# CogSP/CoEvoNet

Measured on AMD Instinct MI355X. Metric: env-steps/sec (agent-steps of the whole job; generations/sec in gens_per_sec), Co-GA simple_adversary_v3 pop=200 HoF=5, higher is better.
Workload: dtype f32

## Files before the change

coevonet_amd/csrc/fc_forward.hip:

```cpp
#include <cstdlib>
#include <type_traits>

#include "coevo_common.hip.h"

namespace coevo {

#ifndef COEVO_HEAVY16_U
#define COEVO_HEAVY16_U 4
#endif
#ifndef COEVO_LIGHT_U
#define COEVO_LIGHT_U 8
#endif

typedef float f32x4_t __attribute__((ext_vector_type(4)));
typedef float f32x4_acc __attribute__((ext_vector_type(4)));
__device__ inline float4 load_stream16(const float4 *p)
{
#ifdef COEVO_NO_NT
    return *p;
#else
    const f32x4_t v = __builtin_nontemporal_load(reinterpret_cast<const f32x4_t *>(p));
    return make_float4(v[0], v[1], v[2], v[3]);
#endif
}
// ... 1054 lines not shown
template <int NB>
__device__ __forceinline__ float mfma16_row_total(const float (*red)[8], int lc, int lg)
{
    const float *rr = red[4 * lg + (lc & 3)];
    const float4 a = *reinterpret_cast<const float4 *>(rr);
    float tot = ((a.x + a.y) + a.z) + a.w;
    if constexpr (NB == 8) {
        const float4 b = *reinterpret_cast<const float4 *>(rr + 4);
        tot = (((tot + b.x) + b.y) + b.z) + b.w;
    }
    return tot;
}
__device__ __forceinline__ void quad_spread(float v, float (&out)[4])
{
    out[0] = dpp_move<0x00>(v); out[1] = dpp_move<0x55>(v); out[2] = dpp_move<0xAA>(v); out[3] = dpp_move<0xFF>(v);
}

template <int MODE>
__device__ __forceinline__ void fc_policy_mfma16_body(const FcArgs &a, FcMfma16Smem &sm, const coevo_fc_task &task)
{
    typedef unsigned u32x2_s __attribute__((ext_vector_type(2)));
    COEVO_STAMP(0);
    const int t = threadIdx.x, w = t >> 6, l = t & 63, lc = l & 15, lg = l >> 4;
    const int D = task.D, nrows = task.n_rows, row0 = task.row_begin;
    const float *net = a.slab + task.net_off;
    int st = 0;

    constexpr int KS = 3;
    float *par = &sm.h1a[0][0];
    {
        const int n_pieces = (D + 3) * (H1 / 4);
#pragma unroll
        for (int j = 0; j < 7; ++j)
            if (64 * w + 256 * j < n_pieces)
                __builtin_amdgcn_global_load_lds((const __attribute__((address_space(1))) void *)(net + 4 * (t + 256 * j)),
                                                 (__attribute__((address_space(3))) void *)(par + 4 * (64 * w + 256 * j)),
                                                 16, 0, 0);
    }
    float p_b2[4], p_g2[4], p_be2[4];
    {
        const float *b2p = net + fc_off_b2(D);
#pragma unroll
        for (int T = 0; T < 4; ++T) p_b2[T] = b2p[64 * w + 16 * T + lc];
    }
    const float p_b3 = (t < 16 * NACT) ? net[fc_off_b3(D) + t % NACT] : 0.0f;

    if constexpr (MODE >= MODE_FUSED) {
// ... 81 lines not shown
        for (int T = 0; T < 8; ++T) c1[T][i] = c1[T][i] - stat[i];
    }
    mfma16_block_sums<8, true>(c1, l, s1);
    mfma16_post_sums<8>(s1, sm.red, w, lc, lg);
    __syncthreads();
    quad_spread(1.0f / __builtin_sqrtf(mfma16_row_total<8>(sm.red, lc, lg) * (1.0f / H1) + LN_EPS), stat);
#pragma unroll
    for (int i = 0; i < 4; ++i) {
        const int row = 4 * lg + i;
        const float rstd = stat[i];
#pragma unroll
        for (int T = 0; T < 8; ++T) {
            const float y = __builtin_fmaf(c1[T][i] * rstd, p_g1[T], p_be1[T]);
            if (row < nrows && bad_post_relu(y)) st |= COEVO_ST_BAD_FC1;
            const int k = 128 * w + 16 * T + lc;
            sm.h1a[k][row ^ ((k >> 2) & 3)] = relu_keep_nan(y);
        }
    }
    asm volatile("" : "+v"(st));
    __syncthreads();
    COEVO_STAMP(2);

    f32x4_acc c2[4];
    {
#pragma unroll
        for (int T = 0; T < 4; ++T)
#pragma unroll
            for (int i = 0; i < 4; ++i) c2[T][i] = p_b2[T];
        const float4 *wp = reinterpret_cast<const float4 *>(net + fc_off_w2(D)) + (size_t)w * 128 * 64 + l;
        constexpr int U = COEVO_HEAVY16_U;
        float4 bufA[U], bufB[U];
        auto issue = [&](float4 (&buf)[U], int kq) {
#pragma unroll
            for (int u = 0; u < U; ++u) buf[u] = wp[(size_t)(kq + u) * 64];
        };
        auto consume = [&](const float4 (&buf)[U], int kq) {
#pragma unroll
            for (int u = 0; u < U; ++u) {
                const int q = kq + u;
                const float av = sm.h1a[4 * q + lg][lc ^ (q & 3)];
                const u32x2_s s02 = __builtin_amdgcn_permlane32_swap(__float_as_uint(buf[u].x), __float_as_uint(buf[u].z), false, false);
                const u32x2_s s13 = __builtin_amdgcn_permlane32_swap(__float_as_uint(buf[u].y), __float_as_uint(buf[u].w), false, false);
                const u32x2_s y01 = __builtin_amdgcn_permlane16_swap(s02[0], s13[0], false, false);
                const u32x2_s y23 = __builtin_amdgcn_permlane16_swap(s02[1], s13[1], false, false);
                c2[0] = __builtin_amdgcn_mfma_f32_16x16x4f32(av, __uint_as_float(y01[0]), c2[0], 0, 0, 0);
                c2[1] = __builtin_amdgcn_mfma_f32_16x16x4f32(av, __uint_as_float(y01[1]), c2[1], 0, 0, 0);
                c2[2] = __builtin_amdgcn_mfma_f32_16x16x4f32(av, __uint_as_float(y23[0]), c2[2], 0, 0, 0);
                c2[3] = __builtin_amdgcn_mfma_f32_16x16x4f32(av, __uint_as_float(y23[1]), c2[3], 0, 0, 0);
            }
        };
        issue(bufA, 0);
        int kq = 0;
        for (; kq < 128 - 2 * U; kq += 2 * U) {
            issue(bufB, kq + U);
            __builtin_amdgcn_sched_barrier(0);
            consume(bufA, kq);
            issue(bufA, kq + 2 * U);
            __builtin_amdgcn_sched_barrier(0);
            consume(bufB, kq + U);
        }
        issue(bufB, kq + U);
        __builtin_amdgcn_sched_barrier(0);
        consume(bufA, kq);
        consume(bufB, kq + U);
    }
    COEVO_STAMP(3);
    float s2[1];
    mfma16_block_sums<4, false>(c2, l, s2);
    mfma16_post_sums<4>(s2, sm.red, w, lc, lg);
    __syncthreads();
    quad_spread(mfma16_row_total<4>(sm.red, lc, lg) * (1.0f / H2), stat);
    __syncthreads();
#pragma unroll
    for (int i = 0; i < 4; ++i) {
#pragma unroll
        for (int T = 0; T < 4; ++T) c2[T][i] = c2[T][i] - stat[i];
    }
    mfma16_block_sums<4, true>(c2, l, s2);
    mfma16_post_sums<4>(s2, sm.red, w, lc, lg);
    __syncthreads();
    quad_spread(1.0f / __builtin_sqrtf(mfma16_row_total<4>(sm.red, lc, lg) * (1.0f / H2) + LN_EPS), stat);
#pragma unroll
    for (int i = 0; i < 4; ++i) {
        const int row = 4 * lg + i;
        const float rstd = stat[i];
#pragma unroll
        for (int T = 0; T < 4; ++T) {
            const float y = __builtin_fmaf(c2[T][i] * rstd, p_g2[T], p_be2[T]);
// ... 668 lines not shown
```

coevonet_amd/csrc/offspring.hip:

```cpp
#include "coevo_common.hip.h"
#include "dqn_common.hip.h"
#include "promote_roles.hip.h"
#include "philox.hip.h"

namespace coevo {

__device__ inline void slab_quad_normals(uint64_t seed, uint32_t slo, uint32_t shi, int64_t s0, int D, int64_t P,
                                         float z[4])
{
    int64_t p[4];
#pragma unroll
    for (int i = 0; i < 4; ++i) p[i] = (s0 + i < P) ? fc_slab_to_flat(s0 + i, D) : -1;
    float zz[4];
    int64_t have = -1;
#pragma unroll
    for (int i = 0; i < 4; ++i) {
        if (p[i] < 0) { z[i] = 0.0f; continue; }
        const int64_t q = p[i] >> 2;
        if (q != have) { philox_normal4(seed, slo, shi, (uint32_t)q, zz); have = q; }
        z[i] = zz[p[i] & 3];
    }
}

__device__ __forceinline__ void fc_perturb_block(const float *parent_slab, const int32_t *parent_idx, float *child_slab,
// ... 191 lines not shown
__global__ __launch_bounds__(256) void ga_promote_kernel(GaPromoteArgs a)
{
    const unsigned y = blockIdx.y;
    const PromoteRole R = PROMOTE_ROLE(a, y);
    float *pop = static_cast<float *>(R.pop), *hof = static_cast<float *>(R.hof), *elite = static_cast<float *>(R.elite);
    const int64_t stride = fc_stride(R.D);
    const int64_t s0 = ((int64_t)blockIdx.x * 256 + threadIdx.x) * 4;
    if (s0 >= stride) return;
    float4 e0;
    if (a.sigma && !R.from_pop) {
        uint32_t shi = a.stream_hi_prev + y;
        if (a.gen_dev) shi += 4u * (uint32_t)(*a.gen_dev - 1);
        e0 = promote_rebuild<0>(elite, R.order, stride, s0, a.E, R.D, a.sigma[y], a.seed, shi);
    } else {
        e0 = R.from_pop ? promote_elites<0>(pop, R.order, elite, stride, s0, a.E)
                        : *reinterpret_cast<const float4 *>(elite + s0);
    }
    promote_hof_shift<1>(hof, stride, s0, a.hof);
    *reinterpret_cast<float4 *>(hof + (int64_t)(a.hof - 1) * stride + s0) = e0;
    if (R.to_pop0) *reinterpret_cast<float4 *>(pop + s0) = e0;
    if (a.tick && blockIdx.x == 0 && blockIdx.y == 0 && threadIdx.x == 0) *a.tick += 1;
}

__device__ __forceinline__ float4 es_chunk_sum(float4 tv, const float *pp, int64_t stride, const float *fitness, int lo, int hi)
{
    const float th[4] = {tv.x, tv.y, tv.z, tv.w};
    float acc[4] = {0.0f, 0.0f, 0.0f, 0.0f};
    typedef float f32x4_nt __attribute__((ext_vector_type(4)));
    constexpr int UE = 16;
    int i = lo;
    for (; i + UE <= hi; i += UE) {
        float4 pv[UE];
#pragma unroll
        for (int u = 0; u < UE; ++u) {
            const f32x4_nt v = __builtin_nontemporal_load(reinterpret_cast<const f32x4_nt *>(pp + (int64_t)(i + u) * stride));
            pv[u] = make_float4(v[0], v[1], v[2], v[3]);
        }
#pragma unroll
        for (int u = 0; u < UE; ++u) {
            const float f = fitness[i + u];
            acc[0] = __builtin_fmaf(f, pv[u].x - th[0], acc[0]);
            acc[1] = __builtin_fmaf(f, pv[u].y - th[1], acc[1]);
            acc[2] = __builtin_fmaf(f, pv[u].z - th[2], acc[2]);
            acc[3] = __builtin_fmaf(f, pv[u].w - th[3], acc[3]);
        }
    }
// ... 224 lines not shown
{
    GaPromoteArgs a{};
    if (!promote_roles(a, roles, n_roles, E, hof, false)) return COEVO_ERR_ARG;
    a.sigma = sigma; a.seed = seed; a.stream_hi_prev = stream_hi_prev; a.gen_dev = gen_dev; a.tick = tick;
    unsigned max_blocks = 0;
    for (int r = 0; r < n_roles; ++r) max_blocks = std::max(max_blocks, quad_blocks(fc_stride(roles[r].D)));
    hipLaunchKernelGGL(ga_promote_kernel, dim3(max_blocks, (unsigned)n_roles), dim3(256), 0, (hipStream_t)stream, a);
    COEVO_HIP_CHECK(hipGetLastError());
    return COEVO_OK;
}

extern "C" int coevo_ga_promote(const coevo_ga_promote_role *roles, int n_roles, int E, int hof, void *stream)
{
    return ga_promote_launch(roles, n_roles, E, hof, nullptr, 0, 0, nullptr, nullptr, stream);
}

extern "C" int coevo_ga_promote_tick(const coevo_ga_promote_role *roles, int n_roles, int E, int hof, int32_t *counter,
                                     void *stream)
{
    if (!counter) return COEVO_ERR_ARG;
    return ga_promote_launch(roles, n_roles, E, hof, nullptr, 0, 0, nullptr, counter, stream);
}

extern "C" int coevo_ga_promote_rebuild(const coevo_ga_promote_role *roles, int n_roles, int E, int hof, const float *sigma,
                                        uint64_t seed, uint32_t stream_hi_prev, const int32_t *gen_dev, void *stream)
{
    if (!sigma) return COEVO_ERR_ARG;
    for (int r = 0; roles && r < n_roles && r < 3; ++r)
        if (!roles[r].elites_from_pop && !roles[r].order) return COEVO_ERR_ARG;
    return ga_promote_launch(roles, n_roles, E, hof, sigma, seed, stream_hi_prev, gen_dev, nullptr, stream);
}

extern "C" int coevo_es_update(float *theta_slab_net, const float *pert_slab, int D, const float *fitness, int n,
                               const float *sigma_dev, float lr, void *stream)
{
    if (!theta_slab_net || !pert_slab || !fitness || !sigma_dev || !fc_dim_ok(D) || n <= 0) return COEVO_ERR_ARG;
    const dim3 grid(quad_blocks(fc_stride(D)));
    hipLaunchKernelGGL(es_update_kernel, grid, dim3(256), 0, (hipStream_t)stream, theta_slab_net, pert_slab, D,
                       fitness, n, sigma_dev, lr);
    COEVO_HIP_CHECK(hipGetLastError());
    return COEVO_OK;
}

static int es_partial_launch(const float *theta_net, const float *pert_slab_local, int ind_first, int64_t stride,
                             const float *fitness_all, int n_total, int chunks_total, int chunk_first, int n_chunks,
                             float *partial, void *stream)
// ... 115 lines not shown
```

coevonet_amd/genetic_algorithm.py:

```python
from __future__ import annotations

import os
import time

import numpy as np
import torch

from . import lib as L
from .fcnetwork import FCNetwork
from .ga_half import HalfGAEngine
from .game_logic import create_agent
from .mpe.simple_adversary import ENV_SEED
from .population import (N_EVAL, RET_SLOT, ROLE_D, ROLES, SIGMA_ATTR, CoGASchedule, CoGATail, NetTable, SlabIO,
                         adapt_mutation_power, captured, co_ga_games, eval_gate_limits, half_route, mean_eval_triple,
                         shard_and_gather, slab_layout)
from .rollout import DeviceRollout, HostEnvRollout, RolloutPlan, effective_steps

ROLE_SLOT = {"agent_0": 1, "agent_1": 2, "adversary_0": 0}


def evaluate_current_weights(agent_0, agent_1, adversary, env, args):
    from .game_logic import play_game
    tot = [0.0, 0.0, 0.0]
    for _ in range(N_EVAL):
# ... 9 lines not shown
    children = []
    for i in range(args.population - 1):
        child = elites[i % args.elites_number].clone(env, args, role)
        child.mutate(sigma)
        children.append(child)
    return children


def small_shard_rows(n_local, hof, cus, pop):
    if n_local >= pop or not 1 <= hof <= 8:
        return 16
    per_cu = 2 if os.environ.get("COEVO_PERSISTENT", "1") != "0" else 1
    if 3 * n_local + 6 * hof * -(-n_local // hof) <= per_cu * cus:
        return hof
    return 16


def cohort_partition(n_local, K):
    bounds = np.array([k * n_local // K for k in range(K + 1)], dtype=np.int64)
    return bounds, np.searchsorted(bounds[1:], np.arange(n_local), side="right").astype(np.int32)


RESIDENT_MB_DEFAULT = 224


def resident_budget_bytes():
    v = os.environ.get("COEVO_RESIDENT_MB", "").strip().lower()
    if v == "all":
        return float("inf")
    return (float(v) if v else RESIDENT_MB_DEFAULT) * 1e6


def resident_enabled(env, heavy_rows, n_local, pop):
    return env == "device" and heavy_rows == 16 and n_local >= pop


def resident_prefix(budget_bytes, fixed_bytes, individual_bytes, bounds):
    K = len(bounds) - 1
    sizes = np.diff(np.asarray(bounds, dtype=np.int64))
    left = budget_bytes - fixed_bytes
    if left <= 0 or K <= 0:
        return np.zeros(K, dtype=np.int64)
    if left == float("inf"):
        return sizes
    return np.minimum(sizes, int(left // (K * individual_bytes)))

# ... 9 lines not shown
                 env_seed=ENV_SEED, rng="device_philox", philox_seed=0, env="device", first_ordinal=1,
                 shard=(0, 1), gather=None, timing_pairs=4096, cohorts=1, gather_packed=None):
        assert 1 <= elites <= pop and hof >= 1
        self.pop, self.hof, self.E = pop, hof, elites
        self.rng_mode, self.philox_seed, self.env_mode = rng, int(philox_seed), env
        self.device = device
        self.rank, self.world = shard
        self.gather = gather
        self.gather_packed = gather_packed
        if self.world > 1 and pop % self.world:
            raise ValueError(f"population {pop} is not divisible by the number of ranks {self.world}")
        self.lo = self.rank * pop // self.world
        self.hi = (self.rank + 1) * pop // self.world
        self.n_local = self.hi - self.lo
        self.T_train = effective_steps(limit_train, max_cycles)
        self.T_eval = effective_steps(limit_eval, max_cycles)
        self.n_cycles = (max(self.T_train, self.T_eval) + 2) // 3
        self.first_ordinal = first_ordinal
        self.env_seed = env_seed
        self.stride = {r: L.fc_slab_stride(ROLE_D[r]) for r in ROLES}
        self.P = {r: L.fc_param_count(ROLE_D[r]) for r in ROLES}
        self.base, total = slab_layout(ROLES, (("pop", pop), ("hof", hof), ("elite", elites), ("stale", 1), ("hof_tmp", hof),
                                               ("elite_prev", elites)), self.stride)
        self.slab = torch.zeros(total, dtype=torch.float32, device=device)
        table = NetTable(self.base, self.stride, ROLE_D)
        games, self.n_main = co_ga_games(table, self.lo, self.hi, hof)
        heavy_rows = int(os.environ.get("COEVO_HEAVY_ROWS", "0"))
        if heavy_rows <= 0:
            cus = torch.cuda.get_device_properties(device).multi_processor_count if (env == "device" and str(device) != "cpu") else 0
            heavy_rows = small_shard_rows(self.n_local, hof, cus, pop) if (cus and cohorts <= 1) else 16
        host_k = int(os.environ.get("COEVO_HOST_COHORTS", "0")) or max(1, min(4, len(games) // 700))
        self.K = max(1, min(int(cohorts) if env == "device" else host_k, self.n_local))
        row_order = "class" if env == "device" else "cohort"
        self._set_cohort_bounds()
        game_cohort = None
        if self.K > 1:
            per_ind = np.repeat(cohort_partition(self.n_local, self.K)[1], self.hof)
            game_cohort = np.concatenate([per_ind, per_ind, per_ind, np.full(N_EVAL, self.K - 1)]).astype(np.int32)
        resident = resident_enabled(env, heavy_rows, self.n_local, pop)

        def resident_nets():
            if not resident:
                return ()
            ind_bytes = sum(4 * self.stride[r] for r in ROLES)
            n = resident_prefix(resident_budget_bytes(), (hof + elites + 1) * ind_bytes, ind_bytes, self.cohort_bounds)
            return [table.ids[("pop", r, self.lo + i)] for r in ROLES for k in range(self.K)
                    for i in range(int(self.cohort_bounds[k]), int(self.cohort_bounds[k]) + int(n[k]))]

        try:
            self.plan = RolloutPlan(np.array(games), table.net_off, table.net_D, device=device, heavy_rows=heavy_rows,
                                    n_cohorts=self.K, game_cohort=game_cohort, row_order=row_order,
                                    resident_nets=resident_nets())
        except ValueError:
            self.K = 1
            self._set_cohort_bounds()
            self.plan = RolloutPlan(np.array(games), table.net_off, table.net_D, device=device, heavy_rows=heavy_rows,
                                    row_order=row_order, resident_nets=resident_nets())
        if env == "device":
            self.ro = DeviceRollout(self.plan, self.slab, env_seed=env_seed, timing_pairs=timing_pairs)
        else:
            self.ro = HostEnvRollout(self.plan, self.slab, env_seed=env_seed)
        f32 = dict(dtype=torch.float32, device=device)
        self.dist_all = torch.zeros(3, pop, **f32)
        self.dist = {r: self.dist_all[i] for i, r in enumerate(ROLES)}
        self.div = {r: torch.zeros(1, **f32) for r in ROLES}
        self.fitness = {r: torch.zeros(pop, **f32) for r in ROLES}
        self.order = {r: torch.zeros(pop, dtype=torch.int32, device=device) for r in ROLES}
        self.sigma = {r: torch.zeros(1, **f32) for r in ROLES}
        self.sigma_prev = {r: torch.zeros(1, **f32) for r in ROLES}
        self.last_reward = torch.zeros(3, pop, 3, dtype=torch.float64, device=device)
        self.pack_local = torch.zeros(3, self.n_local, 4, dtype=torch.float64, device=device)
        self.pack_all = torch.zeros(self.world, 3, self.n_local, 4, dtype=torch.float64, device=device)
        self.parent_idx = torch.tensor([c % elites for c in range(max(pop - 1, 1))], dtype=torch.int32, device=device)
        self.hof_shift_idx = torch.arange(1, max(hof, 2), dtype=torch.int32, device=device)
        self.iota = torch.arange(max(hof, elites, 2), dtype=torch.int32, device=device)
        self.generation = 0
        self.steps_per_generation = 3 * pop * hof * self.T_train + N_EVAL * self.T_eval

    def _uploaded(self, region):
        if region in ("pop", "stale"):
            self._dist_current = False

    def download(self, role, region, first, n):
        if region == "pop":
            self.flush_breeding()
        return super().download(role, region, first, n)

    def eval_rewards(self):
        self.ro.check_status()
        if hasattr(self.ro, "collect_stamps"):
            self.ro.collect_stamps()
        return mean_eval_triple(self.rewards_host()[self.n_main:])

    def select(self):
        if torch.is_tensor(self.ro.rewards):
            dev_rewards = self.ro.rewards
        else:
            if getattr(self, "_rewards_dev", None) is None:
                self._rewards_pin = torch.zeros(self.plan.n_games, 3, dtype=torch.float64).pin_memory()
                self._rewards_dev = torch.zeros(self.plan.n_games, 3, dtype=torch.float64, device=self.device)
            self._rewards_pin.numpy()[:] = self.ro.rewards
            self._rewards_dev.copy_(self._rewards_pin, non_blocking=True)
            dev_rewards = self._rewards_dev
        per_phase = self.n_local * self.hof
# ... 177 lines not shown
        if tick:
            L.call("coevo_counter_add", L._p(self.gen_dev), 1)

    def _reset_cohort(self, k, gen):
        lo_k, hi_k = self._cohort_individuals(k)
        base, M = self._ordinal_base(gen), 3 * self.pop * self.hof
        per_phase = self.n_local * self.hof
        segs = [(ph * per_phase + (lo_k - self.lo) * self.hof, (hi_k - lo_k) * self.hof,
                 base + ph * self.pop * self.hof + lo_k * self.hof) for ph in range(3)]
        if k == self.K - 1 and gen > 0:
            segs.append((self.n_main, N_EVAL, self._ordinal_base(gen - 1) + M))
        self.ro.reset_segments(segs, arm=(k, self.n_cycles))

    def flush_breeding(self):
        if getattr(self, "_breeding_pending", False):
            torch.cuda.synchronize()
            for k in range(self.K):
                self._breed_cohort(k, self.generation_enqueued - 1)
            torch.cuda.synchronize()
            self._breeding_pending = False

    def replay_generation_pipelined(self, gen):
        assert self.world == 1 and self.env_mode == "device" and self.fused_tail and self.K > 1
        self._enqueue_cohort_chains(gen)
        if self._tail_graph is None:
            self._tail_graph = captured(lambda: self._enqueue_selection_and_breeding(breed=False))
        self._tail_graph.replay()
        self._breeding_pending = self.pop > 1
        self.generation_enqueued = gen + 1

    def _enqueue_cohort_chains(self, gen):
        ro = self.ro
        if gen <= 1:
            ro.set_limits(eval_gate_limits(self.plan.n_games, self.n_main, self.T_train, self.T_eval, gen))
        main = torch.cuda.current_stream()
        if getattr(self, "_cohort_streams", None) is None:
            self._cohort_streams = [main] + [
                torch.cuda.ExternalStream(L.load().coevo_rollout_ctx_cohort_stream(ro.ctx, k), device=self.device)
                for k in range(1, self.K)]
            self._cohort_done = [torch.cuda.Event() for _ in range(self.K)]
            self._tail_done = torch.cuda.Event()
            self._tail_graph = None
            self._breeding_pending = False
        self._tail_done.record(main)
        for k, s in reversed(list(enumerate(self._cohort_streams))):
            if k:
# ... 353 lines not shown
```

coevonet_amd/lib.py:

```python
from __future__ import annotations

import ctypes as C
import os

import numpy as np
import torch

HERE = os.path.dirname(os.path.abspath(__file__))
LIB_PATH = os.environ.get("COEVO_LIB") or os.path.join(HERE, "libcoevo.so")

OBS_STRIDE = 12
LOGIT_STRIDE = 8
FC_MAX_ROWS = 32
MPE_STATE_DOUBLES = 24
STAMP_SLOTS = 32
ST_NAMES = {1: "input contains inf or NaN", 2: "output contains inf or NaN after fc1",
            4: "output contains inf or NaN after fc2", 8: "output contains inf or NaN",
            16: "no action selected (current_best_position = -1)",
            32: "persistent rollout: a workgroup timed out waiting for the other rows of its games (COEVO_ST_SYNC_TIMEOUT)",
            64: "fp16 forward: a task with a bad width, row count or unaligned net offset was skipped (COEVO_ST_BAD_TASK)"}

DQN_LOGIT_STRIDE = 32
DQN_FC1_TILED = 0x100
DQP_SKIP_BN = 1
DQN_MAX_ROWS = 16
DQN_TASK_DTYPE = np.dtype([("net_off", "<i8"), ("row_begin", "<i4"), ("n_rows", "<i4")])

TASK_DTYPE = np.dtype([("net_off", "<i8"), ("row_begin", "<i4"), ("n_rows", "<i4"), ("D", "<i4"),
                       ("reserved", "<i4")])
TASK_RESIDENT = 1


class PCG64State(C.Structure):
    _fields_ = [("state_hi", C.c_uint64), ("state_lo", C.c_uint64), ("inc_hi", C.c_uint64), ("inc_lo", C.c_uint64)]

    @classmethod
    def from_seed(cls, seed):
        st = np.random.PCG64(seed).state["state"]
        m = (1 << 64) - 1
        return cls(st["state"] >> 64, st["state"] & m, st["inc"] >> 64, st["inc"] & m)


class PerturbJob(C.Structure):
    _fields_ = [("parent_slab", C.c_void_p), ("parent_idx", C.c_void_p), ("child_slab", C.c_void_p),
                ("sigma_dev", C.c_void_p), ("dist_ref", C.c_void_p), ("dist_partial", C.c_void_p),
                ("child_first", C.c_int32), ("n_children", C.c_int32), ("D", C.c_int32),
                ("stream_lo_first", C.c_uint32), ("stream_hi", C.c_uint32), ("pad", C.c_int32)]


class Perturb16Job(C.Structure):
    _fields_ = list(PerturbJob._fields_)


# ... 101 lines not shown
    "coevo_fc16_distance": (C.c_int, [C.c_void_p, C.c_void_p, C.c_int, C.c_int, C.c_void_p, C.c_void_p]),
    "coevo_fc16_distance_finalize": (C.c_int, [C.c_void_p, C.c_int, C.c_int, C.c_void_p, C.c_int, C.c_void_p,
                                               C.c_void_p]),
    "coevo_fc16_perturb_dist_multi": (C.c_int, [C.c_void_p, C.c_int, C.c_uint64, C.c_int, C.c_void_p, C.c_void_p]),
    "coevo_fc16_distance_finalize_multi": (C.c_int, [C.c_void_p, C.c_int, C.c_void_p]),
    "coevo_fc16_gather": (C.c_int, [C.c_void_p, C.c_void_p, C.c_void_p, C.c_int, C.c_int, C.c_int, C.c_void_p]),
    "coevo_ga16_promote": (C.c_int, [C.c_void_p, C.c_int, C.c_int, C.c_int, C.c_void_p]),
    "coevo_es16_partial_floats": (C.c_int64, [C.c_int]),
    "coevo_es16_fitness": (C.c_int, [C.c_void_p, C.c_void_p, C.c_int, C.c_int, C.c_void_p, C.c_void_p, C.c_void_p]),
    "coevo_es16_partial": (C.c_int, [C.c_int, C.c_void_p, C.c_int, C.c_int, C.c_void_p, C.c_uint64, C.c_uint32, C.c_uint32,
                                     C.c_void_p, C.c_void_p]),
    "coevo_es16_apply": (C.c_int, [C.c_void_p, C.c_void_p, C.c_int, C.c_int, C.c_int, C.c_void_p, C.c_double, C.c_void_p]),
    "coevo_fc_forward_merged": (C.c_int, [C.c_void_p, C.c_void_p, C.c_int, C.c_int, C.c_void_p, C.c_int, C.c_int, C.c_void_p,
                                         C.c_void_p, C.c_void_p, C.c_void_p, C.c_void_p]),
    "coevo_mpe_reset": (C.c_int, [C.c_void_p, C.c_int, C.c_int, C.c_int, PCG64State, C.c_uint64, C.c_void_p]),
    "coevo_mpe_reset_multi": (C.c_int, [C.c_void_p, C.c_int, C.c_void_p, C.c_int, PCG64State, C.c_void_p]),
    "coevo_mpe_reset_multi_arm": (C.c_int, [C.c_void_p, C.c_int, C.c_void_p, C.c_int, PCG64State, C.c_void_p, C.c_int,
                                            C.c_void_p]),
    "coevo_mpe_reset_multi_prep": (C.c_int, [C.c_void_p, C.c_int, C.c_void_p, C.c_int, PCG64State, C.c_void_p, C.c_int,
                                             C.c_void_p, C.c_int, C.c_void_p]),
    "coevo_ga_select_adapt": (C.c_int, [C.c_void_p, C.c_int, C.c_int, C.c_int, C.c_int, C.c_void_p, C.c_int, C.c_void_p,
                                        C.c_void_p]),
    "coevo_ga_promote_tick": (C.c_int, [C.c_void_p, C.c_int, C.c_int, C.c_int, C.c_void_p, C.c_void_p]),
    "coevo_fc_perturb_dist_multi": (C.c_int, [C.c_void_p, C.c_int, C.c_uint64, C.c_int, C.c_void_p, C.c_void_p]),
    "coevo_fc_distance_finalize_multi": (C.c_int, [C.c_void_p, C.c_int, C.c_void_p]),
    "coevo_mpe_reset_gen": (C.c_int, [C.c_void_p, C.c_int, C.c_int, C.c_int, PCG64State, C.c_int64, C.c_void_p,
                                      C.c_int64, C.c_void_p]),
    "coevo_mpe_observe": (C.c_int, [C.c_void_p, C.c_int, C.c_void_p, C.c_void_p, C.c_int, C.c_void_p, C.c_void_p]),
    "coevo_mpe_step": (C.c_int, [C.c_void_p, C.c_int, C.c_void_p, C.c_void_p, C.c_int, C.c_void_p, C.c_int,
                                 C.c_void_p]),
    "coevo_mpe_host_reset": (C.c_int, [C.c_void_p, C.c_int, PCG64State, C.c_void_p]),
    "coevo_mpe_host_reset_games": (C.c_int, [C.c_void_p, C.c_int, PCG64State, C.c_void_p, C.c_void_p, C.c_int, C.c_int]),
    "coevo_mpe_host_observe": (C.c_int, [C.c_void_p, C.c_int, C.c_void_p, C.c_void_p, C.c_int, C.c_void_p]),
    "coevo_mpe_host_step": (C.c_int, [C.c_void_p, C.c_int, C.c_void_p, C.c_void_p, C.c_int, C.c_int, C.c_void_p, C.c_int]),
    "coevo_mpe_host_step_games": (C.c_int, [C.c_void_p, C.c_int, C.c_void_p, C.c_void_p, C.c_int, C.c_void_p, C.c_int,
                                            C.c_void_p, C.c_int, C.c_int, C.c_int, C.c_void_p]),
    "coevo_host_rollout_create": (C.c_void_p, [C.c_int, C.c_int]),
    "coevo_host_rollout_destroy": (None, [C.c_void_p]),
    "coevo_host_rollout_threads": (C.c_int, [C.c_void_p]),
    "coevo_host_rollout_step": (C.c_int, [C.c_void_p, C.c_void_p, C.c_int, C.c_void_p, C.c_void_p, C.c_int, C.c_int,
                                          C.c_void_p, C.c_int, C.c_void_p, C.c_int, C.c_int, C.c_void_p]),
    "coevo_mpe_host_rollout": (C.c_int, [C.c_void_p, C.POINTER(HostRolloutDesc), C.c_void_p]),
    "coevo_host_placement_choose": (C.c_int, [C.c_char_p, C.c_char_p, C.c_char_p, C.c_char_p, C.c_int, C.c_int, C.c_int,
                                              C.c_void_p, C.c_void_p]),
    "coevo_host_rollout_placement": (C.c_int, [C.c_void_p, C.c_void_p, C.c_int, C.c_void_p]),
    "coevo_host_rollout_alloc": (C.c_void_p, [C.c_void_p, C.c_size_t]),
# ... 222 lines not shown
```

coevonet_amd/population.py:

```python
from __future__ import annotations

import os

import numpy as np
import torch

from . import lib as L
from .rollout import DeviceRollout, RolloutPlan

ROLES = ("agent_0", "agent_1", "adversary_0")
ROLE_D = {"agent_0": 10, "agent_1": 10, "adversary_0": 8}
RET_SLOT = {"agent_0": 0, "agent_1": 1, "adversary_0": 2}
ROLES2 = ("first_0", "second_0")
N_EVAL = 10
ES_CHUNKS = 8
SIGMA_ATTR = {"agent_0": "mutation_power_agent_0", "agent_1": "mutation_power_agent_1",
              "adversary_0": "mutation_power_adversary"}


def slab_layout(roles, regions, stride_of):
    base, off = {}, 0
    for r in roles:
        base[r] = {}
        for region, count in regions:
# ... 198 lines not shown
    _perturb_dist_entry = "coevo_fc_perturb_dist"
    _finalize_entry = "coevo_fc_distance_finalize"

    def _select_roles(self, rewards_ptr_of, game_first_of, games_per_individual):
        roles = (L.GaSelectRole * 3)()
        for ri, r in enumerate(ROLES):
            roles[ri] = L.GaSelectRole(L._p(self.dist[r]), rewards_ptr_of(ri), L._p(self.div[r]), L._p(self.fitness[r]),
                                       L._p(self.order[r]), L._p(self.best_dist[r]), game_first_of(ri), RET_SLOT[r])
        L.call("coevo_ga_select", roles, 3, self.pop, games_per_individual, self.hof)

    def _select_unfused(self, rewards_ptr_of, game_first_of, games_per_individual):
        for ri, r in enumerate(ROLES):
            L.call("coevo_sharing_score", L._p(self.dist[r]), self.pop, L._p(self.div[r]))
            L.call("coevo_ga_fitness", rewards_ptr_of(ri), game_first_of(ri), self.pop, games_per_individual, self.hof,
                   RET_SLOT[r], L._p(self.div[r]), L._p(self.fitness[r]))
            L.call("coevo_rank_desc", L._p(self.fitness[r]), self.pop, L._p(self.order[r]))

    def _promote_roles(self, elites_from_pop, best_to_pop0, tick=False, rebuild=None):
        roles = (L.GaPromoteRole * 3)()
        for ri, r in enumerate(ROLES):
            roles[ri] = L.GaPromoteRole(self._ptr(r, "pop"), self._ptr(r, "hof"), self._ptr(r, "elite"),
                                        L._p(self.order[r]), ROLE_D[r], 1 if elites_from_pop else 0,
                                        1 if best_to_pop0 else 0, 0)
        if rebuild is not None:
            L.call("coevo_ga_promote_rebuild", roles, 3, self.E, self.hof, L._p(self.sigma32_prev), self.philox_seed, *rebuild)
        elif tick:
            L.call("coevo_ga_promote_tick", roles, 3, self.E, self.hof, L._p(self.gen_dev))
        else:
            L.call(self._promote_entry, roles, 3, self.E, self.hof)

    def _elites_unfused(self, r, rebuild=None):
        D = ROLE_D[r]
        if rebuild is None:
            L.call("coevo_fc_gather", self._ptr(r, "pop"), L._p(self.order[r]), self._ptr(r, "elite"), 0, self.E, D)
            return
        sigma_ptr, stream, gen_ptr = rebuild
        L.call("coevo_fc_gather", self._ptr(r, "elite"), L._p(self.iota), self._ptr(r, "elite_prev"), 0, self.E, D)
        L.call("coevo_fc_rebuild_elites", self._ptr(r, "elite_prev"), L._p(self.order[r]), self._ptr(r, "elite"), self.E, D,
               sigma_ptr, self.philox_seed, stream, gen_ptr)

    def _hof_push(self, r):
        D = ROLE_D[r]
        if self.hof > 1:
            L.call("coevo_fc_gather", self._ptr(r, "hof"), L._p(self.hof_shift_idx), self._ptr(r, "hof_tmp"), 0,
                   self.hof - 1, D)
            L.call("coevo_fc_gather", self._ptr(r, "hof_tmp"), L._p(self.iota), self._ptr(r, "hof"), 0,
                   self.hof - 1, D)
        L.call("coevo_fc_gather", self._ptr(r, "elite"), L._p(self.iota), self._ptr(r, "hof"), self.hof - 1, 1, D)

    def _best_to_pop0(self, r):
        L.call("coevo_fc_gather", self._ptr(r, "elite"), L._p(self.iota), self._ptr(r, "pop"), 0, 1, ROLE_D[r])

    def _promote_unfused(self, r, best_to_pop0=True, best_dist=False):
        self._hof_push(r)
        if best_to_pop0:
            self._best_to_pop0(r)
        if best_dist:
            L.call("coevo_gather_f32", L._p(self.best_dist[r]), L._p(self.dist[r]), L._p(self.order[r]), 1)

    def _breed_role_children(self, ri, r, c_lo, c_hi, stream, gen_dev, sigma_ptr):
        L.call(self._perturb_dist_entry, self._ptr(r, "elite"), self.parent_idx.data_ptr() + 4 * c_lo, self._ptr(r, "pop"),
               1 + c_lo, c_hi - c_lo, ROLE_D[r], sigma_ptr, self.philox_seed, c_lo, stream, 0, gen_dev, self._ptr(r, "stale"),
               L._p(self.dist_partial[r]))
        L.call(self._finalize_entry, L._p(self.dist_partial[r]), self.pblocks[r], c_hi - c_lo, L._p(self.dist[r]), 1 + c_lo,
               L._p(self.best_dist[r]) if c_lo == 0 else None)


class CoESSchedule:

    def _rollout_pair(self, games, eval_games, table, env_seed, cls=DeviceRollout, host_cohorts=None, **ro_kw):
        cohorts = int(os.environ.get("COEVO_ES_COHORTS", "2")) if host_cohorts is None else host_cohorts
# ... 145 lines not shown
```

include/coevo.h:

```cpp
#ifndef COEVO_H
#define COEVO_H

#include <stddef.h>
#include <stdint.h>

#ifdef __cplusplus
extern "C" {
#endif

#define COEVO_VERSION 103

#define COEVO_OK 0
#define COEVO_ERR_ARG (-1)
#define COEVO_ERR_HIP (-2)
#define COEVO_ERR_UNSUPPORTED (-3)

#define COEVO_ST_BAD_INPUT 1
#define COEVO_ST_BAD_FC1 2
#define COEVO_ST_BAD_FC2 4
#define COEVO_ST_BAD_OUT 8
#define COEVO_ST_NO_ACTION 16
#define COEVO_ST_SYNC_TIMEOUT 32
#define COEVO_ST_BAD_TASK 64

// ... 5 lines not shown
#define COEVO_FC_MAX_ROWS 32
#define COEVO_STAMP_SLOTS 32

#define COEVO_SLOT_ADVERSARY 0
#define COEVO_SLOT_AGENT_0 1
#define COEVO_SLOT_AGENT_1 2

int coevo_version(void);
const char *coevo_build_flags(void);

int64_t coevo_fc_param_count(int D);
int64_t coevo_fc_slab_stride(int D);
int coevo_fc_pack(const float *flat, float *slab, int n, int D, void *stream);
int coevo_fc_unpack(const float *slab, float *flat, int n, int D, void *stream);

typedef struct {
    int64_t net_off;
    int32_t row_begin;
    int32_t n_rows;
    int32_t D;
    int32_t reserved;
} coevo_fc_task;
#define COEVO_TASK_RESIDENT 1

int coevo_fc_forward_argmax(const float *slab, const coevo_fc_task *tasks, int n_tasks, int max_rows_per_task,
                            const float *obs, int32_t *actions, float *logits, int32_t *status, void *stream);
int coevo_fc_forward_merged(const float *slab, const coevo_fc_task *heavy_tasks, int n_heavy, int heavy_max_rows,
                            const coevo_fc_task *light_tasks, int n_light, int light_max_rows, const float *obs,
                            int32_t *actions, float *logits, int32_t *status, void *stream);

int64_t coevo_fc16_slab_stride(int D);
int coevo_fc16_pack(const float *flat, void *slab, int n, int D, void *stream);
int coevo_fc16_unpack(const void *slab, float *flat, int n, int D, void *stream);
int coevo_fc16_forward_argmax(const void *slab, const coevo_fc_task *tasks, int n_tasks, int max_rows_per_task,
                              const float *obs, int32_t *actions, float *logits, int32_t *status, void *stream);

#define COEVO_MPE_STATE_DOUBLES 24
typedef struct {
    uint64_t pcg_state_hi, pcg_state_lo, pcg_inc_hi, pcg_inc_lo;
} coevo_pcg64;

int coevo_mpe_reset(double *state, int n_games, int game_first, int count, coevo_pcg64 rng, uint64_t first_ordinal,
                    void *stream);
typedef struct { int32_t game_first, count; uint64_t first_ordinal; } coevo_reset_seg;
int coevo_mpe_reset_multi(double *state, int n_games, const coevo_reset_seg *segs , int n_segs,
                          coevo_pcg64 rng, void *stream);
// ... 193 lines not shown
    float *fitness;
    int32_t *order;
    float *best_dist;
    int32_t game_first;
    int32_t slot;
} coevo_ga_select_role;
int coevo_ga_select(const coevo_ga_select_role *roles, int n_roles, int pop, int games_per_individual, int hof,
                    void *stream);
int coevo_ga_select_gathered(const coevo_ga_select_role *roles, int n_roles, int pop, int hof, const double *gathered,
                             int n_local, void *stream);
typedef struct coevo_ga_adapt_args {
    const double *rewards; const int32_t *gen_dev; double *hist; double *sig_hist; double *sigma64; float *sigma32;
    float *sigma32_prev; double sig_min, sig_max; int32_t eval_first_game, cap, adaptive, reserved;
} coevo_ga_adapt_args;
int coevo_ga_select_adapt(const coevo_ga_select_role *roles, int n_roles, int pop, int games_per_individual, int hof,
                          const double *gathered, int n_local, const coevo_ga_adapt_args *adapt, void *stream);
typedef struct coevo_ga_promote_role {
    float *pop, *hof, *elite;
    const int32_t *order;
    int32_t D, elites_from_pop, best_to_pop0, reserved;
} coevo_ga_promote_role;
int coevo_ga_promote(const coevo_ga_promote_role *roles, int n_roles, int E, int hof, void *stream);
int coevo_ga_promote_tick(const coevo_ga_promote_role *roles, int n_roles, int E, int hof, int32_t *counter, void *stream);
int coevo_ga_promote_rebuild(const coevo_ga_promote_role *roles, int n_roles, int E, int hof, const float *sigma,
                             uint64_t seed, uint32_t stream_hi_prev, const int32_t *gen_dev, void *stream);
int coevo_fc_gather(const float *src_slab, const int32_t *src_idx, float *dst_slab, int dst_first, int n, int D,
                    void *stream);

int64_t coevo_fc16_perturb_blocks(int D);
int coevo_fc16_perturb_dist(const void *parent_slab, const int32_t *parent_idx, void *child_slab, int child_first,
                            int n_children, int D, const float *sigma_dev, uint64_t seed, uint32_t stream_lo_first,
                            uint32_t stream_hi, int flags, const int32_t *gen_dev, const void *dist_ref,
                            double *dist_partial, void *stream);
int coevo_fc16_distance(const void *ref_net, const void *pop_slab, int n, int D, double *dist_partial, void *stream);
int coevo_fc16_distance_finalize(const double *dist_partial, int n_blocks, int n, float *dist, int first, const float *head,
                                 void *stream);
typedef struct {
    const void *parent_slab; const int32_t *parent_idx; void *child_slab; const float *sigma_dev;
    const void *dist_ref; double *dist_partial;
    int32_t child_first, n_children, D; uint32_t stream_lo_first, stream_hi; int32_t pad;
} coevo_fc16_perturb_job;
int coevo_fc16_perturb_dist_multi(const coevo_fc16_perturb_job *jobs , int n_jobs, uint64_t seed, int flags,
                                  const int32_t *gen_dev, void *stream);
int coevo_fc16_distance_finalize_multi(const coevo_fc_finalize_job *jobs , int n_jobs, void *stream);
int coevo_fc16_gather(const void *src_slab, const int32_t *src_idx, void *dst_slab, int dst_first, int n, int D, void *stream);
typedef struct coevo_ga16_promote_role {
// ... 145 lines not shown
```

Before: 150.0 million.

## Keep tile-major twin copies of hall-of-fame FC2 weights to skip lane permutes

Adds a second copy of each hall-of-fame net's FC2 weight matrix, stored in a tile-major order that matches the MFMA operand layout. Heavy forward tasks that evaluate HoF nets are flagged to read this twin, so they feed MFMAs directly and skip the permlane32/permlane16 swap sequence. The twins are kept in sync by a new promote kernel that shifts them alongside the HoF, plus refresh calls on other update paths. This costs extra device memory, extra writes during promotion and more bookkeeping, and any update path that misses a refresh would read stale weights.

```diff
diff --git a/coevonet_amd/csrc/fc_forward.hip b/coevonet_amd/csrc/fc_forward.hip
--- a/coevonet_amd/csrc/fc_forward.hip
+++ b/coevonet_amd/csrc/fc_forward.hip
@@ -1100,7 +1100,7 @@
     typedef unsigned u32x2_s __attribute__((ext_vector_type(2)));
     COEVO_STAMP(0);
     const int t = threadIdx.x, w = t >> 6, l = t & 63, lc = l & 15, lg = l >> 4;
-    const int D = task.D, nrows = task.n_rows, row0 = task.row_begin;
+    const int D = task.D, nrows = task.n_rows, row0 = task.row_begin, flags = task.reserved;
     const float *net = a.slab + task.net_off;
     int st = 0;
 
@@ -1228,12 +1228,14 @@
     COEVO_STAMP(2);
 
     f32x4_acc c2[4];
-    {
-#pragma unroll
-        for (int T = 0; T < 4; ++T)
-#pragma unroll
-            for (int i = 0; i < 4; ++i) c2[T][i] = p_b2[T];
-        const float4 *wp = reinterpret_cast<const float4 *>(net + fc_off_w2(D)) + (size_t)w * 128 * 64 + l;
+#pragma unroll
+    for (int T = 0; T < 4; ++T)
+#pragma unroll
+        for (int i = 0; i < 4; ++i) c2[T][i] = p_b2[T];
+    auto fc2 = [&](auto tiled) {
+        constexpr bool TILED = decltype(tiled)::value;
+        const float *w2 = TILED ? a.slab + (int64_t)(flags >> COEVO_TASK_TWIN_SHIFT) * COEVO_TASK_TWIN_UNIT : net + fc_off_w2(D);
+        const float4 *wp = reinterpret_cast<const float4 *>(w2) + (size_t)w * 128 * 64 + l;
         constexpr int U = COEVO_HEAVY16_U;
         float4 bufA[U], bufB[U];
         auto issue = [&](float4 (&buf)[U], int kq) {
@@ -1245,14 +1247,21 @@
             for (int u = 0; u < U; ++u) {
                 const int q = kq + u;
                 const float av = sm.h1a[4 * q + lg][lc ^ (q & 3)];
-                const u32x2_s s02 = __builtin_amdgcn_permlane32_swap(__float_as_uint(buf[u].x), __float_as_uint(buf[u].z), false, false);
-                const u32x2_s s13 = __builtin_amdgcn_permlane32_swap(__float_as_uint(buf[u].y), __float_as_uint(buf[u].w), false, false);
-                const u32x2_s y01 = __builtin_amdgcn_permlane16_swap(s02[0], s13[0], false, false);
-                const u32x2_s y23 = __builtin_amdgcn_permlane16_swap(s02[1], s13[1], false, false);
-                c2[0] = __builtin_amdgcn_mfma_f32_16x16x4f32(av, __uint_as_float(y01[0]), c2[0], 0, 0, 0);
-                c2[1] = __builtin_amdgcn_mfma_f32_16x16x4f32(av, __uint_as_float(y01[1]), c2[1], 0, 0, 0);
-                c2[2] = __builtin_amdgcn_mfma_f32_16x16x4f32(av, __uint_as_float(y23[0]), c2[2], 0, 0, 0);
-                c2[3] = __builtin_amdgcn_mfma_f32_16x16x4f32(av, __uint_as_float(y23[1]), c2[3], 0, 0, 0);
+                if constexpr (TILED) {
+                    c2[0] = __builtin_amdgcn_mfma_f32_16x16x4f32(av, buf[u].x, c2[0], 0, 0, 0);
+                    c2[1] = __builtin_amdgcn_mfma_f32_16x16x4f32(av, buf[u].y, c2[1], 0, 0, 0);
+                    c2[2] = __builtin_amdgcn_mfma_f32_16x16x4f32(av, buf[u].z, c2[2], 0, 0, 0);
+                    c2[3] = __builtin_amdgcn_mfma_f32_16x16x4f32(av, buf[u].w, c2[3], 0, 0, 0);
+                } else {
+                    const u32x2_s s02 = __builtin_amdgcn_permlane32_swap(__float_as_uint(buf[u].x), __float_as_uint(buf[u].z), false, false);
+                    const u32x2_s s13 = __builtin_amdgcn_permlane32_swap(__float_as_uint(buf[u].y), __float_as_uint(buf[u].w), false, false);
+                    const u32x2_s y01 = __builtin_amdgcn_permlane16_swap(s02[0], s13[0], false, false);
+                    const u32x2_s y23 = __builtin_amdgcn_permlane16_swap(s02[1], s13[1], false, false);
+                    c2[0] = __builtin_amdgcn_mfma_f32_16x16x4f32(av, __uint_as_float(y01[0]), c2[0], 0, 0, 0);
+                    c2[1] = __builtin_amdgcn_mfma_f32_16x16x4f32(av, __uint_as_float(y01[1]), c2[1], 0, 0, 0);
+                    c2[2] = __builtin_amdgcn_mfma_f32_16x16x4f32(av, __uint_as_float(y23[0]), c2[2], 0, 0, 0);
+                    c2[3] = __builtin_amdgcn_mfma_f32_16x16x4f32(av, __uint_as_float(y23[1]), c2[3], 0, 0, 0);
+                }
             }
         };
         issue(bufA, 0);
@@ -1269,7 +1278,11 @@
         __builtin_amdgcn_sched_barrier(0);
         consume(bufA, kq);
         consume(bufB, kq + U);
-    }
+    };
+    if (!(flags & COEVO_TASK_TILED))
+        fc2(std::false_type{});
+    else
+        fc2(std::true_type{});
     COEVO_STAMP(3);
     float s2[1];
     mfma16_block_sums<4, false>(c2, l, s2);
diff --git a/coevonet_amd/csrc/offspring.hip b/coevonet_amd/csrc/offspring.hip
--- a/coevonet_amd/csrc/offspring.hip
+++ b/coevonet_amd/csrc/offspring.hip
@@ -237,6 +237,57 @@
     if (a.tick && blockIdx.x == 0 && blockIdx.y == 0 && threadIdx.x == 0) *a.tick += 1;
 }
 
+constexpr int64_t W2_FLOATS = (int64_t)H1 * H2;
+__device__ __forceinline__ float4 w2_twin_piece(const float *w2, int64_t t0)
+{
+    const int64_t group = t0 & ~(int64_t)255;
+    const int l = (int)(t0 >> 2) & 63, lc = l & 15, lg = l >> 4;
+    const float *p = w2 + group + 4 * lc + lg;
+    return make_float4(p[0], p[64], p[128], p[192]);
+}
+
+__global__ __launch_bounds__(256) void fc_w2_tile_major_kernel(const float *src, float *dst, int64_t stride, int64_t o_w2)
+{
+    const int64_t t0 = ((int64_t)blockIdx.x * 256 + threadIdx.x) * 4;
+    *reinterpret_cast<float4 *>(dst + (int64_t)blockIdx.y * W2_FLOATS + t0) = w2_twin_piece(src + (int64_t)blockIdx.y * stride + o_w2, t0);
+}
+
+template <int I>
+__device__ __forceinline__ void promote_twin_shift(float *twin, int64_t t0, int n)
+{
+    if constexpr (I < PROMOTE_MAX_HOF) {
+        const float4 v = *reinterpret_cast<const float4 *>(twin + (int64_t)(I < n ? I : n - 1) * W2_FLOATS + t0);
+        promote_twin_shift<I + 1>(twin, t0, n);
+        if (I < n) *reinterpret_cast<float4 *>(twin + (int64_t)(I - 1) * W2_FLOATS + t0) = v;
+    }
+}
+
+__global__ __launch_bounds__(256) void ga_promote_tiled_kernel(GaPromoteArgs a, float *twins)
+{
+    const unsigned y = blockIdx.y;
+    const PromoteRole R = PROMOTE_ROLE(a, y);
+    float *pop = static_cast<float *>(R.pop), *hof = static_cast<float *>(R.hof), *elite = static_cast<float *>(R.elite);
+    const int64_t stride = fc_stride(R.D);
+    const int64_t s0 = ((int64_t)blockIdx.x * 256 + threadIdx.x) * 4;
+    if (s0 >= stride) return;
+    const int64_t t0 = s0 - fc_off_w2(R.D);
+    const bool in_w2 = t0 >= 0 && t0 < W2_FLOATS;
+    float *twin = twins + (int64_t)y * a.hof * W2_FLOATS;
+    float4 tw = make_float4(0.f, 0.f, 0.f, 0.f);
+    if (in_w2) {
+        const float *best = R.from_pop ? pop + (int64_t)R.order[0] * stride : elite;
+        tw = w2_twin_piece(best + fc_off_w2(R.D), t0);
+        promote_twin_shift<1>(twin, t0, a.hof);
+    }
+    const float4 e0 = R.from_pop ? promote_elites<0>(pop, R.order, elite, stride, s0, a.E)
+                                 : *reinterpret_cast<const float4 *>(elite + s0);
+    promote_hof_shift<1>(hof, stride, s0, a.hof);
+    *reinterpret_cast<float4 *>(hof + (int64_t)(a.hof - 1) * stride + s0) = e0;
+    if (R.to_pop0) *reinterpret_cast<float4 *>(pop + s0) = e0;
+    if (in_w2) *reinterpret_cast<float4 *>(twin + (int64_t)(a.hof - 1) * W2_FLOATS + t0) = tw;
+    if (a.tick && blockIdx.x == 0 && blockIdx.y == 0 && threadIdx.x == 0) *a.tick += 1;
+}
+
 __device__ __forceinline__ float4 es_chunk_sum(float4 tv, const float *pp, int64_t stride, const float *fitness, int lo, int hi)
 {
     const float th[4] = {tv.x, tv.y, tv.z, tv.w};
@@ -507,6 +558,30 @@
     return ga_promote_launch(roles, n_roles, E, hof, nullptr, 0, 0, nullptr, counter, stream);
 }
 
+extern "C" int coevo_ga_promote_tick_tiled(const coevo_ga_promote_role *roles, int n_roles, int E, int hof, int32_t *counter,
+                                           float *w2_twins, void *stream)
+{
+    if (!counter || !w2_twins || !aligned16(w2_twins)) return COEVO_ERR_ARG;
+    GaPromoteArgs a{};
+    if (!promote_roles(a, roles, n_roles, E, hof, true)) return COEVO_ERR_ARG;
+    a.tick = counter;
+    unsigned max_blocks = 0;
+    for (int r = 0; r < n_roles; ++r) max_blocks = std::max(max_blocks, quad_blocks(fc_stride(roles[r].D)));
+    hipLaunchKernelGGL(ga_promote_tiled_kernel, dim3(max_blocks, (unsigned)n_roles), dim3(256), 0, (hipStream_t)stream, a, w2_twins);
+    COEVO_HIP_CHECK(hipGetLastError());
+    return COEVO_OK;
+}
+
+extern "C" int coevo_fc_w2_tile_major(const float *src, float *dst, int n_nets, int D, void *stream)
+{
+    if (!src || !dst || !aligned16(src) || !aligned16(dst) || !fc_dim_ok(D) || n_nets < 0 || n_nets > 65535) return COEVO_ERR_ARG;
+    if (n_nets == 0) return COEVO_OK;
+    hipLaunchKernelGGL(fc_w2_tile_major_kernel, dim3((unsigned)(W2_FLOATS / 1024), (unsigned)n_nets), dim3(256), 0,
+                       (hipStream_t)stream, src, dst, fc_stride(D), fc_off_w2(D));
+    COEVO_HIP_CHECK(hipGetLastError());
+    return COEVO_OK;
+}
+
 extern "C" int coevo_ga_promote_rebuild(const coevo_ga_promote_role *roles, int n_roles, int E, int hof, const float *sigma,
                                         uint64_t seed, uint32_t stream_hi_prev, const int32_t *gen_dev, void *stream)
 {
diff --git a/coevonet_amd/genetic_algorithm.py b/coevonet_amd/genetic_algorithm.py
--- a/coevonet_amd/genetic_algorithm.py
+++ b/coevonet_amd/genetic_algorithm.py
@@ -55,6 +55,8 @@
 
 
 RESIDENT_MB_DEFAULT = 224
+
+HOF_TILED_DEFAULT = "1"
 
 
 def resident_budget_bytes():
@@ -110,7 +112,15 @@
         self.P = {r: L.fc_param_count(ROLE_D[r]) for r in ROLES}
         self.base, total = slab_layout(ROLES, (("pop", pop), ("hof", hof), ("elite", elites), ("stale", 1), ("hof_tmp", hof),
                                                ("elite_prev", elites)), self.stride)
-        self.slab = torch.zeros(total, dtype=torch.float32, device=device)
+        self._hof_tiled, self.hof_twin = False, None
+        if env == "device" and self.world == 1 and hof <= 16 and os.environ.get("COEVO_HOF_TILED", HOF_TILED_DEFAULT) != "0":
+            twin0 = -(-total // L.TASK_TWIN_UNIT) * L.TASK_TWIN_UNIT
+            store = torch.zeros(twin0 + 3 * hof * L.W2_FLOATS, dtype=torch.float32, device=device)
+            self.slab, self.hof_twin = store[:total], store[twin0:]
+            self._twin_off = {self.base[r]["hof"] + j * self.stride[r]: twin0 + (ri * hof + j) * L.W2_FLOATS
+                              for ri, r in enumerate(ROLES) for j in range(hof)}
+        else:
+            self.slab = torch.zeros(total, dtype=torch.float32, device=device)
         table = NetTable(self.base, self.stride, ROLE_D)
         games, self.n_main = co_ga_games(table, self.lo, self.hi, hof)
         heavy_rows = int(os.environ.get("COEVO_HEAVY_ROWS", "0"))
@@ -131,7 +141,11 @@
             if not resident:
                 return ()
             ind_bytes = sum(4 * self.stride[r] for r in ROLES)
-            n = resident_prefix(resident_budget_bytes(), (hof + elites + 1) * ind_bytes, ind_bytes, self.cohort_bounds)
+            fixed = (hof + elites + 1) * ind_bytes
+            if self.hof_twin is not None:
+                twin_bytes = 4 * self.hof_twin.numel()
+                fixed += twin_bytes - 3 * hof * 4 * L.W2_FLOATS
+            n = resident_prefix(resident_budget_bytes(), fixed, ind_bytes, self.cohort_bounds)
             return [table.ids[("pop", r, self.lo + i)] for r in ROLES for k in range(self.K)
                     for i in range(int(self.cohort_bounds[k]), int(self.cohort_bounds[k]) + int(n[k]))]
 
@@ -168,6 +182,26 @@
     def _uploaded(self, region):
         if region in ("pop", "stale"):
             self._dist_current = False
+        if region == "hof" and self._hof_tiled:
+            self._refresh_hof_twins()
+
+    def _refresh_hof_twins(self):
+        for ri, r in enumerate(ROLES):
+            L.call("coevo_fc_w2_tile_major", self._ptr(r, "hof"),
+                   self.hof_twin.data_ptr() + 4 * ri * self.hof * L.W2_FLOATS, self.hof, ROLE_D[r])
+
+    def _enable_hof_tiled(self):
+        plan = self.plan
+        torch.cuda.synchronize()
+        self._refresh_hof_twins()
+        tasks = plan.heavy_np.copy()
+        for i, off in enumerate(tasks["net_off"].tolist()):
+            if off in self._twin_off:
+                tasks["reserved"][i] |= L.task_tiled_flags(self._twin_off[off])
+        plan.heavy_np = tasks
+        plan.heavy.copy_(L.tasks_to_device(tasks, self.device))
+        torch.cuda.synchronize()
+        self._hof_tiled = True
 
     def download(self, role, region, first, n):
         if region == "pop":
@@ -391,6 +425,8 @@
 
     def replay_generation_pipelined(self, gen):
         assert self.world == 1 and self.env_mode == "device" and self.fused_tail and self.K > 1
+        if self.hof_twin is not None and not self._hof_tiled and self.plan.heavy is not None:
+            self._enable_hof_tiled()
         self._enqueue_cohort_chains(gen)
         if self._tail_graph is None:
             self._tail_graph = captured(lambda: self._enqueue_selection_and_breeding(breed=False))
diff --git a/coevonet_amd/lib.py b/coevonet_amd/lib.py
--- a/coevonet_amd/lib.py
+++ b/coevonet_amd/lib.py
@@ -29,6 +29,12 @@
 TASK_DTYPE = np.dtype([("net_off", "<i8"), ("row_begin", "<i4"), ("n_rows", "<i4"), ("D", "<i4"),
                        ("reserved", "<i4")])
 TASK_RESIDENT = 1
+TASK_TILED, TASK_TWIN_SHIFT, TASK_TWIN_UNIT, W2_FLOATS = 2, 8, 1024, 512 * 256
+
+
+def task_tiled_flags(twin_off):
+    assert twin_off % TASK_TWIN_UNIT == 0 and 0 <= twin_off // TASK_TWIN_UNIT < 1 << (31 - TASK_TWIN_SHIFT)
+    return TASK_TILED | (twin_off // TASK_TWIN_UNIT) << TASK_TWIN_SHIFT
 
 
 class PCG64State(C.Structure):
@@ -176,6 +182,8 @@
     "coevo_ga_select_adapt": (C.c_int, [C.c_void_p, C.c_int, C.c_int, C.c_int, C.c_int, C.c_void_p, C.c_int, C.c_void_p,
                                         C.c_void_p]),
     "coevo_ga_promote_tick": (C.c_int, [C.c_void_p, C.c_int, C.c_int, C.c_int, C.c_void_p, C.c_void_p]),
+    "coevo_ga_promote_tick_tiled": (C.c_int, [C.c_void_p, C.c_int, C.c_int, C.c_int, C.c_void_p, C.c_void_p, C.c_void_p]),
+    "coevo_fc_w2_tile_major": (C.c_int, [C.c_void_p, C.c_void_p, C.c_int, C.c_int, C.c_void_p]),
     "coevo_fc_perturb_dist_multi": (C.c_int, [C.c_void_p, C.c_int, C.c_uint64, C.c_int, C.c_void_p, C.c_void_p]),
     "coevo_fc_distance_finalize_multi": (C.c_int, [C.c_void_p, C.c_int, C.c_void_p]),
     "coevo_mpe_reset_gen": (C.c_int, [C.c_void_p, C.c_int, C.c_int, C.c_int, PCG64State, C.c_int64, C.c_void_p,
diff --git a/coevonet_amd/population.py b/coevonet_amd/population.py
--- a/coevonet_amd/population.py
+++ b/coevonet_amd/population.py
@@ -244,12 +244,18 @@
             roles[ri] = L.GaPromoteRole(self._ptr(r, "pop"), self._ptr(r, "hof"), self._ptr(r, "elite"),
                                         L._p(self.order[r]), ROLE_D[r], 1 if elites_from_pop else 0,
                                         1 if best_to_pop0 else 0, 0)
+        tiled = getattr(self, "_hof_tiled", False)
+        if tick and rebuild is None and tiled:
+            L.call("coevo_ga_promote_tick_tiled", roles, 3, self.E, self.hof, L._p(self.gen_dev), L._p(self.hof_twin))
+            return
         if rebuild is not None:
             L.call("coevo_ga_promote_rebuild", roles, 3, self.E, self.hof, L._p(self.sigma32_prev), self.philox_seed, *rebuild)
         elif tick:
             L.call("coevo_ga_promote_tick", roles, 3, self.E, self.hof, L._p(self.gen_dev))
         else:
             L.call(self._promote_entry, roles, 3, self.E, self.hof)
+        if tiled:
+            self._refresh_hof_twins()
 
     def _elites_unfused(self, r, rebuild=None):
         D = ROLE_D[r]
@@ -269,6 +275,8 @@
             L.call("coevo_fc_gather", self._ptr(r, "hof_tmp"), L._p(self.iota), self._ptr(r, "hof"), 0,
                    self.hof - 1, D)
         L.call("coevo_fc_gather", self._ptr(r, "elite"), L._p(self.iota), self._ptr(r, "hof"), self.hof - 1, 1, D)
+        if getattr(self, "_hof_tiled", False):
+            self._refresh_hof_twins()
 
     def _best_to_pop0(self, r):
         L.call("coevo_fc_gather", self._ptr(r, "elite"), L._p(self.iota), self._ptr(r, "pop"), 0, 1, ROLE_D[r])
diff --git a/include/coevo.h b/include/coevo.h
--- a/include/coevo.h
+++ b/include/coevo.h
@@ -51,6 +51,11 @@
     int32_t reserved;
 } coevo_fc_task;
 #define COEVO_TASK_RESIDENT 1
+#define COEVO_TASK_TILED 2
+#define COEVO_TASK_TWIN_SHIFT 8
+#define COEVO_TASK_TWIN_UNIT 1024
+#define COEVO_FC_W2_FLOATS (COEVO_FC_H1 * COEVO_FC_H2)
+int coevo_fc_w2_tile_major(const float *src, float *dst, int n_nets, int D, void *stream);
 
 int coevo_fc_forward_argmax(const float *slab, const coevo_fc_task *tasks, int n_tasks, int max_rows_per_task,
                             const float *obs, int32_t *actions, float *logits, int32_t *status, void *stream);
@@ -290,6 +295,8 @@
 } coevo_ga_promote_role;
 int coevo_ga_promote(const coevo_ga_promote_role *roles, int n_roles, int E, int hof, void *stream);
 int coevo_ga_promote_tick(const coevo_ga_promote_role *roles, int n_roles, int E, int hof, int32_t *counter, void *stream);
+int coevo_ga_promote_tick_tiled(const coevo_ga_promote_role *roles, int n_roles, int E, int hof, int32_t *counter,
+                                float *w2_twins, void *stream);
 int coevo_ga_promote_rebuild(const coevo_ga_promote_role *roles, int n_roles, int E, int hof, const float *sigma,
                              uint64_t seed, uint32_t stream_hi_prev, const int32_t *gen_dev, void *stream);
 int coevo_fc_gather(const float *src_slab, const int32_t *src_idx, float *dst_slab, int dst_first, int n, int D,
```

After: 153.1 million (median of 6 runs). +2.0%, better.
